# davidfischinger/haf_grasping

Hardware: AMD Instinct MI355X
Metric: grid-cell x rotation SVM evals/sec (higher is better)
Workload: dtype f16

## Files before the change

haf_grasping_amd/capi.py:

```python
import ctypes as C
import os

import numpy as np

HERE = os.path.dirname(os.path.abspath(__file__))
LIB_PATH = os.environ.get("HAF_LIB", os.path.join(HERE, "libhafgrasp.so"))
TESTLIB_PATH = os.environ.get("HAF_TESTLIB", os.path.join(HERE, "libhafgrasp_testing.so"))

HAF_OK, HAF_E_ARG, HAF_E_IO, HAF_E_DEVICE, HAF_E_CAPACITY, HAF_E_BUDGET, HAF_E_INTERNAL = 0, -1, -2, -3, -4, -5, -6
FLAG_KEEP_DEBUG, FLAG_PROFILE, FLAG_FP32_MFMA, FLAG_SPLIT_F16, FLAG_PROBABILITY, FLAG_FULL_RANK = 1, 2, 4, 8, 16, 32
DBG_HEIGHTS, DBG_INTEGRAL, DBG_MASK, DBG_LABELS, DBG_DECISION, DBG_TRANSFORM, DBG_SCREEN_MARGIN, DBG_PROBABILITY, DBG_GRASPSGRID, DBG_ROI = range(10)
SHARD_ROLLS, SHARD_CLOUDS = 0, 1
FRAME_DEPTH_U16, FRAME_DEPTH_F32, FRAME_XYZ_F32 = 0, 1, 2
MAP_NO_CELL = -32768
MAX_LABELS = 4096
STAGES = ["upload", "bin", "integral", "mask", "features", "svm", "refine", "recheck", "vote", "download"]


class Config(C.Structure):
    _fields_ = [("feature_file", C.c_char_p), ("range_file", C.c_char_p), ("model_file", C.c_char_p),
                ("nr_features_without_shaf", C.c_int32), ("grid_h", C.c_int32), ("grid_w", C.c_int32),
                ("n_rolls", C.c_int32), ("roll_step_deg", C.c_int32), ("z_shift", C.c_float),
                ("graspval_top", C.c_int32), ("device", C.c_int32), ("max_clouds", C.c_int32),
                ("max_points", C.c_int64), ("flags", C.c_uint32), ("graspval_th", C.c_int32),
# ... 229 lines not shown
        L.haf_test_roll_geo.argtypes = [C.POINTER(Config), C.POINTER(GraspInput), C.c_int, C.c_void_p, C.c_void_p,
                                        C.c_void_p]
        L.haf_test_finalize.argtypes = [C.POINTER(Config), C.POINTER(GraspInput), C.c_void_p, C.POINTER(GraspOutput)]
        L.haf_test_roll_pose.argtypes = [C.POINTER(Config), C.POINTER(GraspInput), C.c_void_p, C.c_int,
                                         C.POINTER(GraspOutput), C.POINTER(C.c_int32)]
        L.haf_test_mfma_kappa.argtypes = [E, C.c_void_p, C.c_void_p]
        L.haf_test_f16_mfma.argtypes = [C.c_void_p, C.c_void_p, C.c_void_p, C.c_void_p, C.c_int, C.c_int]
        L.haf_test_screen_state.argtypes = [E, C.POINTER(C.c_int), C.POINTER(C.c_int), C.POINTER(C.c_double)]
        L.haf_test_set_screen_inactive.argtypes = [E]
        L.haf_test_check_canaries.argtypes = [C.c_char_p, C.c_int]
        L.haf_test_canary_buffers.argtypes = []
        L.haf_test_poke_flag0_list.argtypes = [E, C.c_int, C.c_int, C.c_int]
        L.haf_test_overflow_stats.argtypes = [E, C.c_void_p]
        L.haf_test_fetch_list.argtypes = [E, C.c_int, C.c_void_p, C.c_int, C.POINTER(C.c_int)]
        L.haf_test_snapshot_screen.argtypes = [E, C.c_int]
        L.haf_test_fetch_snapshot.argtypes = [E, C.c_int, C.c_longlong, C.c_void_p, C.c_longlong, C.POINTER(C.c_longlong)]
        L.haf_test_tier_plan.argtypes = [C.c_void_p, C.c_int, C.c_void_p, C.c_int, C.c_int]
        L.haf_test_revote.argtypes = [E, C.c_void_p, C.c_void_p, C.c_void_p, C.c_void_p, C.c_void_p]
        L.haf_test_last_batch.argtypes = [E, C.POINTER(C.c_int), C.POINTER(C.c_int)]
        L.haf_test_top_merge.argtypes = [C.POINTER(Config), C.POINTER(GraspInput), C.c_int] + [C.c_void_p] * 5 + \
            [C.c_int, C.c_int, C.c_double, C.c_void_p, C.POINTER(C.c_int32), C.POINTER(C.c_int32)]
    return L


def lib():
    global _lib
    if _lib is None:
        _lib = _bind(LIB_PATH, testing=False)
    return _lib

# ... 440 lines not shown
        a, b, c = C.c_int32(), C.c_int32(), C.c_int32()
        self._check(self._L.haf_model_info(self._h, C.byref(a), C.byref(b), C.byref(c)))
        return dict(n_sv=a.value, dim=b.value, n_features=c.value)

    def last_counts(self):
        a, r, b, c = C.c_int64(), C.c_int64(), C.c_int64(), C.c_int64()
        self._check(self._L.haf_last_tiers(self._h, C.byref(a), C.byref(r), C.byref(b), C.byref(c)))
        return dict(n_evals=a.value, n_refined=r.value, n_rechecked=b.value, n_strict=c.value)

    def fetch_list(self, which, cap=1 << 22):
        buf = np.empty(cap, dtype=np.int32)
        n = C.c_int()
        self._check(self._L.haf_test_fetch_list(self._h, which, buf.ctypes.data_as(C.c_void_p), cap, C.byref(n)))
        return buf[:min(n.value, cap)].copy()

    def snapshot_screen(self, on=True):
        self._check(self._L.haf_test_snapshot_screen(self._h, 1 if on else 0))

    def fetch_snapshot(self, which, offset=0, nbytes=None):
        avail = C.c_longlong()
        self._check(self._L.haf_test_fetch_snapshot(self._h, which, 0, None, 0, C.byref(avail)))
        if nbytes is None:
            nbytes = avail.value - offset
        buf = np.empty(max(0, nbytes), dtype=np.uint8)
        if nbytes > 0:
            self._check(self._L.haf_test_fetch_snapshot(self._h, which, offset, buf.ctypes.data_as(C.c_void_p), nbytes, C.byref(avail)))
        return buf

    def revote(self, labels=None, gridf=None, heights=None, roi_words=None):
        H, W = self.cfg.grid_h, self.cfg.grid_w
# ... 373 lines not shown
```

haf_grasping_amd/csrc/engine_request.cpp:

```cpp
#include "engine_state.h"

namespace haf_host {

static double host_kernel_value(const SvmModel &m, const double *xg, int n, int kx)
{
    double acc = 0.0;
    if (m.kernel_type == HAF_KERNEL_RBF) {
        for (int k = 0; k < kx; k++) {
            const double sv = k < m.dim ? m.sv[(size_t)n * m.dim + k] : 0.0;
            const double dd = xg[(size_t)k * 16] - sv;
            acc += dd * dd;
        }
        return std::exp(-m.gamma * acc);
    }
    for (int k = 0; k < kx; k++) {
        const double sv = k < m.dim ? m.sv[(size_t)n * m.dim + k] : 0.0;
        acc += xg[(size_t)k * 16] * sv;
    }
    if (m.kernel_type == HAF_KERNEL_POLY) {
        double tmp = m.gamma * acc + m.coef0, ret = 1.0;
        for (int t = m.degree; t > 0; t /= 2) { if (t % 2 == 1) ret *= tmp; tmp = tmp * tmp; }
        return ret;
    }
    if (m.kernel_type == HAF_KERNEL_SIGMOID) return std::tanh(m.gamma * acc + m.coef0);
// ... 133 lines not shown
    p.i8 = f.i8_active && !f.small_exact && !cr_poly_t1;
    if (p.i8) { p.i8_in = L_FLAG; p.i8_out = L_FLAGI; }
    p.fp64 = f.small_exact ? FP64_SMALL : FP64_MFMA;
    p.fp64_in = p.i8 ? L_FLAGI : L_FLAG;
    p.fp64_out = L_FLAG2;
    p.pass0_out = L_FLAG;
    if (p.path != PATH_SCREEN) return p;

    p.cr = v == SCREEN_CR_EXP || v == SCREEN_CR_POLY;
    p.reuse = f.reuse_operands;
    const bool lr_plain = v == SCREEN_PLAIN && f.lr_plain_available;
    p.lr = (p.cr || lr_plain) && f.large && f.lr_available && f.lr_enabled && !f.fused_pre && f.hw > 8192 && !f.reuse_operands;
    p.sp = p.lr && lr_plain ? SP_LRP : p.cr ? SP_CR : SP_PLAIN;
    if (f.use_t0b && f.cr_available && !f.small_exact && (!p.cr || (p.lr && v == SCREEN_CR_EXP)))
        p.t0b = p.sp == SP_LRP && f.lr_fused && !f.t0b_no_gather ? T0B_GATHER : T0B_FEATURES;
    const bool straight = f.small_exact || f.t1_skip;
    if (p.t0b != T0B_NONE) {
        p.pass0_out = L_FLAG0;
        p.t0b_in = L_FLAG0;
        p.t0b_out = straight ? L_FLAG : L_FLAG0B;
    } else {
        p.pass0_out = straight ? L_FLAG : L_FLAG0;
    }
    p.t1 = !straight;
    if (!p.t1) return p;
    p.t1_in = p.t0b != T0B_NONE ? L_FLAG0B : L_FLAG0;
    p.t1_cnt = list_counter(p.t1_in);
    p.t1_out = L_FLAG;
    p.t1cr = cr_poly_t1;
    p.gate = f.calibrated && f.short_gate && f.n_sv >= kShortGateMinSv && f.evals_cap <= 65536;
// ... 21 lines not shown
    int n_frames = 0;
    FrameDev *h_frames = nullptr;
    const FrameDev *d_frames = nullptr;
    RoiViewDev *h_roi_views = nullptr;
    const RoiViewDev *d_roi_views = nullptr;
    std::vector<LastCall::CloudSrc> src;
    CloudDev *h_clouds = nullptr;
    const CloudDev *d_clouds = nullptr;
    const RollGeo *d_geo = nullptr;
    hipStream_t s = nullptr;
    Dims d{};
    float r_row = 0.0f, r_col = 0.0f;
    long evals_cap = 0, evals_sel = 0;
    bool direct = false, short_request = false, small_exact = false, large = false, fused_pre = false;
    bool i8_used = false, t0b_used = false;
    bool lr_used = false;
    int host_resolved = 0;
};

static int check_request(haf_engine *e, int32_t n_clouds, const haf_cloud *clouds, const haf_grasp_input *in, int32_t roll_first,
                         int32_t roll_count, const haf_roll_record *records, Request &q)
{
    if (!clouds || !in || !records || n_clouds < 1) return fail(e, HAF_E_ARG, "haf_score_rolls: null or empty argument");
    const haf_config &c = e->cfg;
    if (n_clouds > c.max_clouds) return fail(e, HAF_E_CAPACITY, "more clouds than max_clouds");
    if (roll_first < 0 || roll_count < 1 || roll_first + roll_count > c.n_rolls) return fail(e, HAF_E_ARG, "roll range outside [0, n_rolls)");
    if (roll_count > e->max_rolls) return fail(e, HAF_E_CAPACITY, "more rolls in one call than max_rolls_per_call");
    HIPCHK(e, hipSetDevice(c.device));
    q.B = n_clouds;
    q.R = roll_count;
// ... 200 lines not shown
        launch_mask_count_roi(e->d_ii.p, q.d_geo, e->d_roi_cells.p, e->d_mask.p, e->d_rowcount.p, d, s);
    } else {
        launch_mask_count(e->d_ii.p, q.d_geo, e->d_mask.p, e->d_rowcount.p, d, s);
    }
    launch_scan(e->d_rowcount.p, e->d_rowoff.p, e->d_brcount.p, e->d_counters.p, d, s);
    launch_compact(e->d_mask.p, e->d_rowcount.p, e->d_rowoff.p, e->d_evalcell.p, d, s);
    if (q.direct) launch_prob_list(e->d_counters.p, CNT_FLAGGED, e->d_flag_list.p, e->list_cap, s);
    return HAF_OK;
}

static TierFacts tier_facts(const haf_engine *e, const Request &q, int mode, bool reuse_operands)
{
    return TierFacts{e->screen_variant, e->cr_available, e->lr_available, e->lr_enabled, e->lr_plain_available, e->lr_fused,
                     e->use_t0b, e->t1_skip, e->t1_cr_available, e->i8_active, e->calibrated, e->short_gate, e->generic_kernel,
                     e->model.n_sv, test_env("HAF_T0B_NO_GATHER") != nullptr, mode, reuse_operands, q.direct, q.small_exact, q.large,
                     q.fused_pre, (long)q.d.H * q.d.W, q.evals_cap};
}

static void launch_screening(haf_engine *e, const Request &q, const TierPlan &p)
{
    const hipStream_t s = q.s;
    const Dims &d = q.d;
    const long evals_cap = q.evals_cap;
    ScreenParams sp_now = p.sp == SP_LRP ? e->screen_lrp : p.sp == SP_CR ? e->screen_cr : e->screen;
    if (p.sp != SP_LRP) sp_now.cr_poly = e->screen_variant == SCREEN_CR_POLY;
    if (p.lr) { sp_now.lr = 1; sp_now.lr_negflags = e->d_inexact.p; sp_now.lr_iiabs = e->d_iiabs.p; }
    if (!p.reuse)
        launch_features(e->d_ii.p, e->d_evalcell.p, e->d_counters.p, e->d_fd.p, e->d_X.p, e->d_gband.p, d, e->range.lower,
                        e->range.upper, e->svm.neg_gamma2, evals_cap, XMODE_SCREEN, sp_now, nullptr, 0, 0, q.large, q.evals_sel, nullptr, e->d_ax.p, s);
    if (e->snap_on && !p.reuse) {
        const long cap = std::min<long>(evals_cap, e->max_evals_pad);
        e->snap_cap = cap;
        (void)hipMemcpyAsync(e->snap_X.p, e->d_X.p, (size_t)((cap + kTile - 1) / kTile) * (size_t)kS0MatBytes, hipMemcpyDeviceToDevice, s);
        (void)hipMemcpyAsync(e->snap_gband.p, e->d_gband.p, (size_t)cap * kBandFloats * sizeof(float), hipMemcpyDeviceToDevice, s);
        (void)hipMemcpyAsync(e->snap_ax.p, e->d_ax.p, (size_t)cap * sizeof(float), hipMemcpyDeviceToDevice, s);
    }
    char *y_img = reinterpret_cast<char *>(e->d_X.p) + (size_t)(e->max_evals_pad / kTile) * (size_t)kS0MatBytes;
    mark(e, HAF_ST_SVM);
    if (p.lr && !e->lr_fused) launch_project(e->d_X.p, e->d_lr_btiles.p, y_img, e->d_gband.p, e->d_counters.p, evals_cap, s);
    if (p.lr)
        launch_svm_screen_lr(e->lr_fused ? reinterpret_cast<char *>(e->d_X.p) : y_img, e->d_gband.p, e->d_ax.p, e->d_svt_lr.p, e->d_evalcell.p, e->d_counters.p, e->svm, e->d_dec.p, e->d_labels.p,
                             e->d_flag0_words.p, e->d_flag0_wgcount.p, list_buf(e, p.pass0_out), e->flag0_cap, e->d_counters.p, d,
                             evals_cap, e->d_margin.p, e->screen_variant, e->crp, e->lr_band, s, handover_counter(p.pass0_out),
                             e->lr_fused ? e->d_lr_btiles_in.p : nullptr);
    else
        launch_svm_screen(e->d_X.p, e->d_gband.p, e->d_ax.p, p.cr ? e->d_svt0_cr.p : e->d_svt0.p, e->d_evalcell.p, e->d_counters.p, e->svm, e->d_dec.p, e->d_labels.p,
                          e->d_flag0_words.p, e->d_flag0_wgcount.p, list_buf(e, p.pass0_out), e->flag0_cap, e->d_counters.p, d, evals_cap, e->d_margin.p,
                          e->screen_variant, e->crp, s, handover_counter(p.pass0_out), nullptr, CNT_EVALS, CNT_FLAGGED0, e->d_screen_part.p, e->screen_parts);
    mark(e, HAF_ST_REFINE);
    const long list_cap = std::min<long>(e->flag0_cap, evals_cap);
    if (p.t0b == T0B_GATHER) {
        launch_svm_screen_lr(reinterpret_cast<char *>(e->d_X.p), e->d_gband.p, e->d_ax.p, e->d_svt_lr.p, e->d_evalcell.p, e->d_counters.p, e->svm, e->d_dec.p,
                             e->d_labels.p, e->d_flag0_words.p, e->d_flag0_wgcount.p, list_buf(e, p.t0b_out), e->flag0_cap,
                             e->d_counters.p, d, list_cap, e->d_margin.p, SCREEN_CR_EXP, e->crp, e->lr_band, s, handover_counter(p.t0b_out),
                             e->d_lr_btiles_in.p, list_buf(e, p.t0b_in), list_counter(p.t0b_in), CNT_FLAGGED0B);
    } else if (p.t0b == T0B_FEATURES) {
        ScreenParams sp_b = e->screen_cr;
        sp_b.cr_poly = 0;
        launch_features(e->d_ii.p, e->d_evalcell.p, e->d_counters.p, e->d_fd.p, e->d_X1.p, e->d_gband.p, d, e->range.lower,
                        e->range.upper, e->svm.neg_gamma2, list_cap, XMODE_SCREEN, sp_b, list_buf(e, p.t0b_in), list_counter(p.t0b_in), e->flag0_cap,
                        false, list_cap, nullptr, e->d_ax.p, s);
        launch_svm_screen(e->d_X1.p, e->d_gband.p, e->d_ax.p, e->d_svt0_cr.p, e->d_evalcell.p, e->d_counters.p, e->svm, e->d_dec.p, e->d_labels.p,
                          e->d_flag0_words.p, e->d_flag0_wgcount.p, list_buf(e, p.t0b_out), e->flag0_cap, e->d_counters.p, d,
                          list_cap, e->d_margin.p, SCREEN_CR_EXP, e->crp, s, handover_counter(p.t0b_out), list_buf(e, p.t0b_in), list_counter(p.t0b_in),
                          CNT_FLAGGED0B, e->d_screen_part.p, e->screen_parts);
    }
    if (p.gate)
        launch_short_list_gate(e->d_counters.p, list_counter(p.gate_in), list_buf(e, p.gate_in), e->flag0_cap, list_buf(e, p.gate_out),
                               CNT_FLAGGEDI, p.gate_out == L_FLAGI, std::min(kShortListGate, e->flag_cap), s);
    if (!p.t1) return;
// ... 117 lines not shown
    }
    return HAF_OK;
}

static int decide(haf_engine *e, Request &q, int mode, bool reuse_operands)
{
    mark(e, HAF_ST_FEATURES);
    const TierPlan p = plan_tiers(tier_facts(e, q, mode, reuse_operands));
    if (p.path == PATH_SCREEN) {
        q.lr_used = p.lr;
        launch_screening(e, q, p);
    } else {
        launch_first_pass(e, q, p);
    }
    q.t0b_used = p.t0b != T0B_NONE;
    q.i8_used = p.i8;
    mark(e, HAF_ST_RECHECK);
    if (p.fp64 != FP64_NONE) {
        if (p.i8) i8_window(e, q, p, 0);
        fp64_window(e, q, p, 0);
    }
    const int rc = vote_and_wait(e, q);
    if (rc != HAF_OK) return rc;
    return finish_exact_tiers(e, q, p);
}

static int decide_probability(haf_engine *e, Request &q)
{
    const hipStream_t s = q.s;
    const Dims &d = q.d;
// ... 84 lines not shown
}

static int record_outcome(haf_engine *e, const Request &q, int mode, int inexact_grids, int roll_first, const haf_grasp_input *in,
                          haf_roll_record *records)
{
    if (e->cfg.flags & HAF_FLAG_PROFILE)
        for (int i = 0; i < HAF_ST_COUNT; i++) (void)hipEventElapsedTime(&e->stage_ms[i], e->ev[i], e->ev[i + 1]);
    const int *h = e->h_counters;
    LastCall &l = e->last;
    l.B = q.B; l.R = q.R; l.roll_first = roll_first;
    l.evals = h[CNT_EVALS];
    l.flagged = e->prob_mode ? 0 : h[CNT_FLAGGED];
    l.flagged2 = h[CNT_FLAGGED2];
    l.lr = q.lr_used;
    l.flagged0 = q.t0b_used ? std::min(h[CNT_FLAGGED0B], h[CNT_FLAGGED0]) : h[CNT_FLAGGED0];
    l.flaggedi = q.i8_used ? h[CNT_FLAGGEDI] : h[CNT_FLAGGED];
    l.bypass = h[CNT_BYPASS];
    l.inexact = inexact_grids;
    l.screened = (mode == MODE_SCREEN) && !e->prob_mode && !q.direct && h[CNT_FLAGGED0] <= e->flag0_cap;
    l.host_resolved = q.host_resolved;
    l.i8 = q.i8_used;
    l.inputs.assign(in, in + q.B);
    l.clouds = q.src;
    l.roi = q.from.roi != nullptr;
    for (int b = 0; q.from.views && b < q.B; b++) l.clouds[(size_t)b].n = (size_t)q.h_clouds[b].n;
    if (hipMemsetAsync(e->d_counters.p, 0, CNT_COUNT * sizeof(int), q.s) == hipSuccess) e->counters_clean = true;
    if (l.flagged > e->list_cap || l.flagged2 > e->list_cap || l.flaggedi > e->list_cap) return fail(e, HAF_E_INTERNAL, "recheck list counters exceed the number of evaluations");
    if (const int rc = check_guards(e)) return rc;
    for (int i = 0; i < q.B * q.R; i++) {
        records[i].vote = e->h_rec[i].vote;
// ... 116 lines not shown
```

haf_grasping_amd/csrc/engine_state.h:

```cpp
#pragma once
#include "../../include/hafgrasp.h"
#include "kernels.h"
#include "parsers.h"
#include "frame_stage.h"
#include "decq.h"
#include "engine_internal.h"

#include <algorithm>
#include <chrono>
#include <cmath>
#include <cstdio>
#include <cstdlib>
#include <cstring>
#include <mutex>
#include <new>
#include <string>
#include <vector>

using namespace haf;

namespace haf_host {

#ifdef HAF_TESTING
inline const char *test_env(const char *name) { return getenv(name); }
// ... 89 lines not shown
        char *h = nullptr;
        hipError_t rc = d.alloc(bytes);
        pinned_failed = rc == hipSuccess && (rc = hipHostMalloc((void **)&h, bytes, hipHostMallocDefault)) != hipSuccess;
        if (rc != hipSuccess) { d.release(); return rc; }
        release();
        dev = d; host = h;
        return hipSuccess;
    }
    void release() { dev.release(); if (host) (void)hipHostFree(host); host = nullptr; }
};

struct LastCall {
    int B = 0, R = 0, roll_first = 0;
    int evals = 0;
    int flagged0 = 0;
    int flagged = 0;
    int flaggedi = 0;
    int bypass = 0;
    int flagged2 = 0;
    int host_resolved = 0;
    int inexact = 0;
    bool screened = false;
    bool lr = false;
    bool i8 = false;
    std::vector<haf_grasp_input> inputs;
    struct CloudSrc { size_t float_off = 0; size_t n = 0; bool staged = false; };
    std::vector<CloudSrc> clouds;
    bool roi = false;
};

// ... 207 lines not shown
inline int list_counter(int l)
{
    static const int cnt[] = {CNT_FLAGGED0, CNT_FLAGGED0B, CNT_FLAGGED, CNT_FLAGGEDI, CNT_FLAGGED2};
    return l == L_NONE ? -1 : cnt[l];
}
struct TierFacts {
    int screen_variant = SCREEN_PLAIN;
    bool cr_available = false, lr_available = false, lr_enabled = false, lr_plain_available = false, lr_fused = false;
    bool use_t0b = false, t1_skip = false, t1_cr_available = false, i8_active = false, calibrated = false, short_gate = false;
    bool generic_kernel = false;
    int n_sv = 0;
    bool t0b_no_gather = false;
    int mode = MODE_SCREEN;
    bool reuse_operands = false, direct = false, small_exact = false, large = false, fused_pre = false;
    long hw = 0, evals_cap = 0;
};
enum { PATH_GENERIC, PATH_DIRECT, PATH_SCREEN, PATH_SPLIT, PATH_F32 };
enum { SP_PLAIN, SP_CR, SP_LRP };
enum { T0B_NONE, T0B_GATHER, T0B_FEATURES };
enum { FP64_NONE, FP64_SMALL, FP64_MFMA };
struct TierPlan {
    int path = PATH_SCREEN;
    int sp = SP_PLAIN;
    bool cr = false, lr = false;
    bool reuse = false;
    int pass0_out = L_NONE;
    int t0b = T0B_NONE, t0b_in = L_NONE, t0b_out = L_NONE;
    bool gate = false;
    int gate_in = L_NONE, gate_out = L_NONE;
    bool t1 = false, t1cr = false;
    int t1_in = L_NONE, t1_cnt = -1, t1_out = L_NONE;
    bool i8 = false;
    int i8_in = L_NONE, i8_out = L_NONE;
    int fp64 = FP64_NONE, fp64_in = L_NONE, fp64_out = L_NONE;
    int strict_in = L_FLAG2;
};
TierPlan plan_tiers(const TierFacts &f);

inline int fail(haf_engine *e, int code, const std::string &msg)
{
    e->error = msg;
    return code;
// ... 63 lines not shown
```

haf_grasping_amd/csrc/engine_testing.cpp:

```cpp
#include "engine_state.h"

#ifndef HAF_TESTING
#error "engine_testing.cpp belongs to the testing build (-DHAF_TESTING)"
#endif

namespace haf_host {
namespace {
struct CanaryRec { char *user; size_t bytes; const char *file; int line; };
std::mutex g_canary_mu;
std::vector<CanaryRec> g_canary;
}
void canary_register(void *user, size_t bytes, const char *file, int line)
{
    std::lock_guard<std::mutex> lk(g_canary_mu);
    g_canary.push_back(CanaryRec{static_cast<char *>(user), bytes, file, line});
}
void canary_unregister(void *user)
{
    std::lock_guard<std::mutex> lk(g_canary_mu);
    for (size_t i = 0; i < g_canary.size(); i++)
        if (g_canary[i].user == user) { g_canary[i] = g_canary.back(); g_canary.pop_back(); return; }
}
int canary_check(std::string *report)
{
// ... 93 lines not shown
    if (!e || !avail || offset < 0 || bytes < 0 || which < 0 || which > 2) return HAF_E_ARG;
    const char *src = which == 0 ? e->snap_X.p : which == 1 ? reinterpret_cast<const char *>(e->snap_gband.p) : reinterpret_cast<const char *>(e->snap_ax.p);
    const long long have = which == 0 ? (long long)((e->snap_cap + kTile - 1) / kTile) * kS0MatBytes
                                      : (long long)e->snap_cap * (which == 1 ? kBandFloats : 1) * (long long)sizeof(float);
    *avail = src ? have : 0;
    if (!bytes) return HAF_OK;
    if (!src || !out || offset + bytes > have) return HAF_E_ARG;
    if (hipDeviceSynchronize() != hipSuccess) return HAF_E_DEVICE;
    return hipMemcpy(out, src + offset, (size_t)bytes, hipMemcpyDeviceToHost) == hipSuccess ? HAF_OK : HAF_E_DEVICE;
}
int haf_test_poke_flag0_list(haf_engine *e, int at, int count, int v)
{
    if (!e || !e->d_flag0_list.p) return HAF_E_ARG;
    std::vector<int> h((size_t)count, v);
    return hipMemcpy(e->d_flag0_list.p + e->d_flag0_list.n + at, h.data(), h.size() * sizeof(int), hipMemcpyHostToDevice) == hipSuccess ? HAF_OK : HAF_E_DEVICE;
}

int haf_test_last_batch(haf_engine *e, int *B, int *R)
{
    if (!e || !B || !R) return HAF_E_ARG;
    *B = e->last.B; *R = e->last.R;
    return HAF_OK;
}

static int revote_impl(haf_engine *e, const int8_t *labels, const float *gridf, const float *heights, const unsigned long long *roi_words,
                       haf_roll_record *records_out)
{
    if (!records_out || (labels != nullptr) == (gridf != nullptr)) return fail(e, HAF_E_ARG, "haf_test_revote: exactly one of labels and gridf, and records_out");
    if ((gridf != nullptr) != e->prob_mode) return fail(e, HAF_E_ARG, "haf_test_revote: labels go with a plain engine, gridf with HAF_FLAG_PROBABILITY");
    if (roi_words && !labels) return fail(e, HAF_E_ARG, "haf_test_revote: roi_words go with labels");
// ... 355 lines not shown
```

haf_grasping_amd/csrc/kernels.h:

```cpp
#pragma once

#include <hip/hip_runtime.h>
#include <stddef.h>
#include <stdint.h>
#include "frame_points.h"
#include "frames.h"
#include "grasp_cells.h"

namespace haf {

constexpr int kKP = 324;
constexpr int kKSteps = kKP / 2;
constexpr int kDP = 328;
constexpr int kTile = 32;
constexpr int kTileFloats = kDP * kTile;
constexpr int kSvmBlockEvals = 256;
constexpr int kSvmThreads = 512;
constexpr int kHListParts = 4;

constexpr int kHK = 336;
constexpr int kHFull = 10;
constexpr int kHSteps = kHK / 16;
constexpr int kHMatBytes = kHSteps * 1024;
constexpr int kHTailOff = kHFull * 2048;
// ... 13 lines not shown
constexpr int kS0WaveEvals = 64;
constexpr int kS0Waves = 4;
constexpr int kS0BlockEvals = kS0Waves * kS0WaveEvals;
constexpr int kS0K = 320;
constexpr int kS0Groups = kS0K / 8;
constexpr int kS0MatBytes = kHFull * 2048;
constexpr int kS0WavePieces = 5;
constexpr int kS0SvTileBytes = 21504;
constexpr int kS0Pieces = kS0SvTileBytes / 1024;
constexpr int kS0Buffers = 3;
constexpr float kF16MinNormal = 6.103515625e-05f;
constexpr int kLrK = 192;
constexpr int kLrSteps = kLrK / 32;
constexpr int kLrMatBytes = kLrSteps * 2048;
constexpr int kLrSvTileBytes = kLrMatBytes + 1024;
constexpr int kLrWavePieces = 3;
constexpr int kLrProjTileBytes = kHFull * 2048;

__host__ __device__ inline double split3_f16(double a, _Float16 out[3])
{
    auto rn = [](double v) {
        _Float16 h = (_Float16)(float)v;
        float f = (float)h;
        if ((f < 0 ? -f : f) < kF16MinNormal) h = (_Float16)0.0f;
        return h;
    };
    out[0] = rn(a);
    const double r1 = a - (double)(float)out[0];
    out[1] = rn(r1 * 4096.0);
    const double r2 = r1 - (double)(float)out[1] / 4096.0;
// ... 239 lines not shown
       XMODE_F64 = 3,
       XMODE_I8 = 4 };
void launch_features(const float *ii, const int *evalcell, const int *counters, const FeatDesc *fd, float *X, float *ax,
                     Dims d, double lower, double upper, float neg_gamma2, long max_evals, int xmode, ScreenParams sp,
                     const int *idx_list, int list_counter, int list_cap, bool large, long sel_evals, AttrRecord *dbg,
                     float *ax2, hipStream_t s,
                     int list_off = 0);
double probe_mfma_rounding(hipStream_t s, double *worst16);
int probe_f16_subnormal_mfma(hipStream_t s);
void launch_project(const void *X0, const void *btiles, void *Y, float *raw, const int *counters, long max_evals, hipStream_t s);
void launch_svm_screen_lr(const void *Y, float *raw, const float *nax, const void *svt_lr, const int *evalcell, const int *counters,
                          SvmParams p, float *dec, int8_t *labels, unsigned long long *flag0_words, int *wgcount, int *flag0_list,
                          int flag0_cap, int *counters_rw, Dims d, long max_evals, float *margin, int variant, CrParams cr, LrBand lb,
                          hipStream_t s, int also_counter = -1,
                          const void *ptiles = nullptr,
                          const int *idx_list = nullptr, int count_slot = CNT_EVALS, int out_slot = CNT_FLAGGED0);
void launch_svm_screen(const void *X0, const float *gband, const float *nax, const void *svt0, const int *evalcell, const int *counters,
                       SvmParams p, float *dec, int8_t *labels, unsigned long long *flag0_words, int *wgcount, int *flag0_list,
                       int flag0_cap, int *counters_rw, Dims d, long max_evals, float *margin, int variant, CrParams cr, hipStream_t s,
                       int also_counter = -1,
                       const int *idx_list = nullptr, int count_slot = CNT_EVALS,
                       int out_slot = CNT_FLAGGED0,
                       void *part_buf = nullptr, int parts = 0);
size_t screen_part_bytes();
void launch_svm(const float *X, const float *ax, const float *svt, const int *evalcell, const int *counters,
                SvmParams p, float *dec, int8_t *labels, int *flag_list, int flag_cap, int *counters_rw, Dims d,
                long max_evals, hipStream_t s,
                unsigned char *t1flags = nullptr);
void launch_short_list_gate(int *counters, int src_slot, const int *src_list, int src_cap, int *dst_list, int dst_slot, bool dst_direct,
                            int max_entries, hipStream_t s);
size_t t1_flag_bytes(long max_entries);
// ... 113 lines not shown
```

haf_grasping_amd/csrc/screen.hip:

```cpp
#include "kernels.h"
#include "screen_band.h"
#include <algorithm>
#include <cmath>
#include <vector>

namespace haf {

typedef float f32x4 __attribute__((ext_vector_type(4)));
typedef _Float16 half8 __attribute__((ext_vector_type(8)));
typedef _Float16 half4 __attribute__((ext_vector_type(4)));

__device__ __forceinline__ void dma_piece(const char *gbase, unsigned lds_dst, unsigned lane16)
{
    asm volatile("s_mov_b32 m0, %0\n\ts_nop 0\n\tglobal_load_lds_dwordx4 %1, %2" ::"s"(lds_dst), "v"(lane16), "s"(gbase) : "memory", "m0");
}

struct TileDma {
    const char *g[kS0WavePieces];
    unsigned l[kS0WavePieces];
};
__device__ __forceinline__ TileDma tile_dma(const char *gtile, unsigned lds_slot, const int (&poff)[kS0WavePieces])
{
    TileDma d;
#pragma unroll
// ... 744 lines not shown
{
    const long blocks = (max_evals + kS0BlockEvals - 1) / kS0BlockEvals;
    if (blocks <= 0) return;
    hipLaunchKernelGGL(k_project, dim3((unsigned)blocks), dim3(kS0Waves * 64), 0, s, (const char *)X0, (const char *)btiles, (char *)Y, raw, counters);
}

#ifndef HAF_LR_WGS
#define HAF_LR_WGS 2
#endif
#ifndef HAF_LR_EXPLAG
#define HAF_LR_EXPLAG 4
#endif
#ifndef HAF_LR_ABL
#define HAF_LR_ABL 0
#endif
constexpr int kLrExpLag = HAF_LR_EXPLAG;
constexpr bool kLrTwoLevel = HAF_LR_WGS < 3;
template <int FIRST, int COUNT, int VAR>
__device__ __forceinline__ void screen_block_lr(const char *cur, int n, int lane, const half8 (&a)[kLrSteps][4], f32x4 (&acc)[4],
                                                const f32x4 (&old)[4], float cf_old, float (&sum)[4][4],
                                                const TileDma &dma, unsigned lane16, half8 &b, half8 &b1)
{
    constexpr bool CRP = VAR == SCREEN_CR_POLY, PLN = VAR == SCREEN_PLAIN;
    static_assert(VAR == SCREEN_CR_EXP || VAR == SCREEN_CR_POLY || VAR == SCREEN_PLAIN, "the low-rank form serves the plain and the centred-remainder variants");
    const char *bl = cur + n * 1024 + lane * 16;
    __builtin_amdgcn_sched_barrier(0);
    const f32x4 z4 = {0.0f, 0.0f, 0.0f, 0.0f};
    const float ba2 = CRP ? cf_old * kPsiA2 : 0.0f, ba3 = CRP ? cf_old * kPsiA3 : 0.0f, ba4 = CRP ? cf_old * kPsiA4 : 0.0f;
    if (n == 0) b = *reinterpret_cast<const half8 *>(bl);
    if (HAF_LR_ABL & 2) asm volatile("" :: "v"(old[0]), "v"(old[1]), "v"(old[2]), "v"(old[3]));
// ... 38 lines not shown
                float ph = fmaf(z, ba4, ba3);
                HAF_SB();
                ph = fmaf(ph, z, ba2);
                HAF_SB();
                sum[e >> 2][e & 3] = fmaf(pt, ph, sum[e >> 2][e & 3]);
                HAF_SB();
            }
        }
        b = b1;
    }
#undef HAF_SB
    __builtin_amdgcn_sched_barrier(0);
}

template <int VAR, bool FUSED, bool GATHER>
__global__ __launch_bounds__(kS0Waves * 64, HAF_LR_WGS) void k_svm_screen_lr(const char *__restrict__ Y, const float *__restrict__ raw,
                                                                  const float *__restrict__ nax, const char *__restrict__ svt,
                                                                  const int *__restrict__ evalcell, const int *__restrict__ counters,
                                                                  SvmParams p, float *__restrict__ dec, int8_t *__restrict__ labels,
                                                                  unsigned long long *__restrict__ flag0_words, Dims d,
                                                                  float *__restrict__ margin, CrParams crp, LrBand lb,
                                                                  const char *__restrict__ ptiles,
                                                                  const int *__restrict__ idx_list, int count_slot, int in_cap)
{
    static_assert(!GATHER || FUSED, "the gather form reads the 10-step images");
    constexpr bool CRP = VAR == SCREEN_CR_POLY;
    constexpr int kV0 = FUSED ? kHFull : 0;
    __shared__ __attribute__((aligned(16))) char lds[kS0Buffers * kLrSvTileBytes + 3 * kS0Waves * kS0WaveEvals * 4];
    const int n_evals = GATHER ? min(counters[count_slot], in_cap) : counters[CNT_EVALS];
    const long base = (long)blockIdx.x * kS0BlockEvals;
    if (base >= n_evals) return;
    const int tid = threadIdx.x, wave = tid >> 6, lane = tid & 63;
    const long tile32 = (base >> 5) + 2 * wave;
    const unsigned lds0 = (unsigned)(uintptr_t)lds;
    const int np = d.sv_tile_neg, nt = d.n_sv_tiles;
    float *pos = reinterpret_cast<float *>(lds + kS0Buffers * kLrSvTileBytes) + wave * kS0WaveEvals;
    float *fin = pos + kS0Waves * kS0WaveEvals;
    float *sdyrow = fin + kS0Waves * kS0WaveEvals;
    const unsigned lane16 = (unsigned)lane * 16u;
    const int wave_u = __builtin_amdgcn_readfirstlane(wave);
    int poff[kS0WavePieces];
// ... 4 lines not shown
        asm volatile("s_nop 4");
#pragma unroll
        for (int q = 0; q < kLrWavePieces; q++) dma_piece(g + poff[q], l + (unsigned)poff[q], lane16);
    };
    auto vtile = [&](int v) -> const char * { return (FUSED && v < kV0) ? ptiles + (size_t)v * kLrMatBytes : svt + (size_t)(v - kV0) * kLrSvTileBytes; };
    {
        stage3(vtile(0), lds0);
        if (!FUSED && wave_u == 0) dma_piece(svt + kLrMatBytes, lds0 + kLrMatBytes, lane16);
    }
    if (FUSED || nt > 1) {
        stage3(vtile(1), lds0 + kLrSvTileBytes);
        if (!FUSED && wave_u == 0) dma_piece(vtile(1) + kLrMatBytes, lds0 + kLrSvTileBytes + kLrMatBytes, lane16);
    }
    half8 a[kLrSteps][4];
    if (!FUSED) {
        const char *xt = Y + (size_t)tile32 * kLrMatBytes;
#pragma unroll
        for (int s = 0; s < kLrSteps; s++)
#pragma unroll
            for (int m = 0; m < 4; m++)
                a[s][m] = __builtin_nontemporal_load(reinterpret_cast<const half8 *>(xt + (m >> 1) * kLrMatBytes + (s * 2 + (m & 1)) * 1024 + lane * 16));
#pragma unroll
        for (int s = 0; s < kLrSteps; s++)
#pragma unroll
            for (int m = 0; m < 4; m++) asm volatile("" : "+v"(a[s][m]));
        asm volatile("s_waitcnt vmcnt(0)" ::: "memory");
        __syncthreads();
    } else {
        const char *xt = Y + (size_t)tile32 * kS0MatBytes;
        const char *xg[4];
        if (GATHER) {
#pragma unroll
            for (int m = 0; m < 4; m++) {
                const long sl = base + wave * kS0WaveEvals + 16 * m + (lane & 15);
                const int eg = sl < n_evals ? idx_list[sl] : 0;
                xg[m] = Y + (size_t)(eg >> 5) * kS0MatBytes + ((eg >> 4) & 1) * 1024 + ((lane >> 4) * 16 + (eg & 15)) * 16;
            }
        }
        auto xload = [&](int sx, half8 (&x)[4]) {
#pragma unroll
            for (int m = 0; m < 4; m++)
                x[m] = GATHER ? *reinterpret_cast<const half8 *>(xg[m] + sx * 2048)
                              : __builtin_nontemporal_load(reinterpret_cast<const half8 *>(xt + (m >> 1) * kS0MatBytes + (sx * 2 + (m & 1)) * 1024 + lane * 16));
        };
        f32x4 accp[2 * kLrSteps][4];
#pragma unroll
        for (int rb = 0; rb < 2 * kLrSteps; rb++)
#pragma unroll
            for (int m = 0; m < 4; m++) accp[rb][m] = f32x4{0.0f, 0.0f, 0.0f, 0.0f};
        half8 xc[4], xn[4];
        xload(0, xc);
#pragma unroll
        for (int m = 0; m < 4; m++) xn[m] = xc[m];
#pragma unroll
        for (int m = 0; m < 4; m++) asm volatile("" : "+v"(xc[m]));
        asm volatile("s_waitcnt vmcnt(0)" ::: "memory");
        __syncthreads();
#pragma unroll 1
        for (int v = 0; v < kV0; v++) {
            const char *cur = lds + (v % kS0Buffers) * kLrSvTileBytes;
#pragma unroll
            for (int rb = 0; rb < 2 * kLrSteps; rb++) {
                const half8 bf = *reinterpret_cast<const half8 *>(cur + rb * 1024 + lane * 16);
                if (!(HAF_LR_ABL & 16)) {
#pragma unroll
                for (int m = 0; m < 4; m++) accp[rb][m] = __builtin_amdgcn_mfma_f32_16x16x32_f16(bf, xc[m], accp[rb][m], 0, 0, 0);
                } else if (rb < 4) {
                    accp[rb][0] = __builtin_amdgcn_mfma_f32_16x16x32_f16(bf, xc[rb], accp[rb][0], 0, 0, 0);
                }
                if (rb == 0) {
                    __builtin_amdgcn_sched_barrier(0);
                    if (v + 1 < kV0) xload(v + 1, xn);
                    const int vn = v + 2;
                    if (vn < kV0 + nt) {
                        const unsigned ls = lds0 + (vn % kS0Buffers) * kLrSvTileBytes;
                        stage3(vtile(vn), ls);
                        if (vn >= kV0 && wave_u == 0) dma_piece(vtile(vn) + kLrMatBytes, ls + kLrMatBytes, lane16);
                    }
                    __builtin_amdgcn_sched_barrier(0);
// ... 112 lines not shown
        const long es = GATHER ? (long)idx_list[e] : e;
        float sc = __builtin_amdgcn_exp2f(nax[es]);
        float4 g, g2 = float4{0.0f, 0.0f, 0.0f, 0.0f};
        float rw[6];
#pragma unroll
        for (int k = 0; k < 6; k++) rw[k] = raw[kBandFloats * es + k];
        if (GATHER) rw[3] = raw[kBandFloats * es + 6];
        if (FUSED) rw[5] = sdyrow[lane];
        if (VAR == SCREEN_PLAIN) lr_finish_band_plain(rw, lb, g, g2);
        else lr_finish_band(rw, lb, g.x, g.y, g.z, g.w);
        asm volatile("s_nop 7\n\ts_nop 7" : "+v"(sc));
        flagged = screen_tail_vals<VAR, false>((double)pos[lane], (double)fin[lane], 0.0f, e, g, g2, sc, p, crp, GATHER ? idx_list : nullptr, evalcell, dec, labels, margin);
    }
    const unsigned long long bal = __ballot(flagged);
    if (lane == 0) flag0_words[(base >> 6) + wave] = bal;
}

void launch_svm_screen(const void *X0, const float *gband, const float *nax, const void *svt0, const int *evalcell, const int *counters,
                       SvmParams p, float *dec, int8_t *labels, unsigned long long *flag0_words, int *wgcount, int *flag0_list,
                       int flag0_cap, int *counters_rw, Dims d, long max_evals, float *margin, int variant, CrParams cr, hipStream_t s,
                       int also_counter, const int *idx_list, int count_slot, int out_slot, void *part_buf, int parts)
{
    long blocks = (max_evals + kS0BlockEvals - 1) / kS0BlockEvals;
    if (blocks <= 0) return;
    const int in_cap = idx_list ? (int)std::min<long>(flag0_cap, max_evals) : 0x7fffffff;
    const bool split = part_buf && parts != 1 && blocks <= kS0PartBlocks && (parts > 1 || d.n_sv_tiles >= 4 * kS0MinPartTiles);
#define HAF_SCREEN_LAUNCH(V)                                                                                                      \
    if (split) {                                                                                                                  \
        hipLaunchKernelGGL((k_svm_screen<V, true>), dim3((unsigned)blocks, kS0MaxParts), dim3(kS0Waves * 64), 0, s, (const char *)X0, gband, nax, \
                           (const char *)svt0, evalcell, counters, p, dec, labels, flag0_words, d, margin, cr, idx_list, count_slot,      \
// ... 6 lines not shown
                           (float4 *)nullptr, 0, in_cap);                                                                         \
    }
    switch (variant) {
        case SCREEN_SUMSQ: HAF_SCREEN_LAUNCH(SCREEN_SUMSQ); break;
        case SCREEN_CR_EXP: HAF_SCREEN_LAUNCH(SCREEN_CR_EXP); break;
        case SCREEN_CR_POLY: HAF_SCREEN_LAUNCH(SCREEN_CR_POLY); break;
        default: HAF_SCREEN_LAUNCH(SCREEN_PLAIN); break;
    }
#undef HAF_SCREEN_LAUNCH
    launch_screen_compaction(flag0_words, wgcount, blocks, flag0_list, flag0_cap, counters_rw, also_counter, idx_list, count_slot, out_slot, in_cap, s);
}

void launch_svm_screen_lr(const void *Y, float *raw, const float *nax, const void *svt_lr, const int *evalcell, const int *counters,
                          SvmParams p, float *dec, int8_t *labels, unsigned long long *flag0_words, int *wgcount, int *flag0_list,
                          int flag0_cap, int *counters_rw, Dims d, long max_evals, float *margin, int variant, CrParams cr, LrBand lb,
                          hipStream_t s, int also_counter, const void *ptiles, const int *idx_list, int count_slot, int out_slot)
{
    const long blocks = (max_evals + kS0BlockEvals - 1) / kS0BlockEvals;
    if (blocks <= 0) return;
    lb.poly = variant == SCREEN_CR_POLY;
    const int in_cap = idx_list ? (int)std::min<long>(flag0_cap, max_evals) : 0x7fffffff;
#define HAF_LR_LAUNCH(V, F, G)                                                                                                        \
    hipLaunchKernelGGL((k_svm_screen_lr<V, F, G>), dim3((unsigned)blocks), dim3(kS0Waves * 64), 0, s, (const char *)Y, raw, nax,        \
                       (const char *)svt_lr, evalcell, counters, p, dec, labels, flag0_words, d, margin, cr, lb, (const char *)ptiles,  \
                       idx_list, count_slot, in_cap)
    if (idx_list) { HAF_LR_LAUNCH(SCREEN_CR_EXP, true, true); }
    else if (variant == SCREEN_CR_POLY) { if (ptiles) HAF_LR_LAUNCH(SCREEN_CR_POLY, true, false); else HAF_LR_LAUNCH(SCREEN_CR_POLY, false, false); }
    else if (variant == SCREEN_PLAIN) { if (ptiles) HAF_LR_LAUNCH(SCREEN_PLAIN, true, false); else HAF_LR_LAUNCH(SCREEN_PLAIN, false, false); }
    else { if (ptiles) HAF_LR_LAUNCH(SCREEN_CR_EXP, true, false); else HAF_LR_LAUNCH(SCREEN_CR_EXP, false, false); }
#undef HAF_LR_LAUNCH
    const int cs = idx_list ? count_slot : CNT_EVALS;
    launch_screen_compaction(flag0_words, wgcount, blocks, flag0_list, flag0_cap, counters_rw, also_counter, idx_list, cs,
                             idx_list ? out_slot : CNT_FLAGGED0, in_cap, s);
}

size_t screen_part_bytes() { return (size_t)kS0MaxParts * kS0PartBlocks * kS0BlockEvals * sizeof(float4); }

}
```

Measured before the change: 540.0 million.

## Store first-pass projected LR features for flagged evals and reuse them in second tier

In the fused plain low-rank screen, each wave now writes its projected f16 feature vectors (and a band value) into a per-eval record buffer, but only for evaluations the first pass flags. The second-tier gather pass then reads these compact records instead of re-gathering from the full 10-step images and re-running the projection MFMAs. The aim is to cut the redundant projection work and bandwidth in the refine screen. In exchange the first pass does extra scattered stores, and it relies on the record buffer aliasing the y_img region. Test hooks and a HAF_T0B_REPROJECT escape are also added.

```diff
diff --git a/haf_grasping_amd/capi.py b/haf_grasping_amd/capi.py
--- a/haf_grasping_amd/capi.py
+++ b/haf_grasping_amd/capi.py
@@ -267,6 +267,8 @@
         L.haf_test_overflow_stats.argtypes = [E, C.c_void_p]
         L.haf_test_fetch_list.argtypes = [E, C.c_int, C.c_void_p, C.c_int, C.POINTER(C.c_int)]
         L.haf_test_snapshot_screen.argtypes = [E, C.c_int]
+        L.haf_test_t0b_state.argtypes = [E, C.c_void_p]
+        L.haf_test_fill_lr_records.argtypes = [E, C.c_int]
         L.haf_test_fetch_snapshot.argtypes = [E, C.c_int, C.c_longlong, C.c_void_p, C.c_longlong, C.POINTER(C.c_longlong)]
         L.haf_test_tier_plan.argtypes = [C.c_void_p, C.c_int, C.c_void_p, C.c_int, C.c_int]
         L.haf_test_revote.argtypes = [E, C.c_void_p, C.c_void_p, C.c_void_p, C.c_void_p, C.c_void_p]
@@ -737,6 +739,14 @@
         self._check(self._L.haf_test_fetch_list(self._h, which, buf.ctypes.data_as(C.c_void_p), cap, C.byref(n)))
         return buf[:min(n.value, cap)].copy()
 
+    def t0b_state(self):
+        out = (C.c_int * 3)()
+        self._check(self._L.haf_test_t0b_state(self._h, out))
+        return dict(first_pass_flagged=int(out[0]), form=("none", "gather", "features")[out[1]], stored=bool(out[2]))
+
+    def fill_lr_records(self, byte=0xFF):
+        self._check(self._L.haf_test_fill_lr_records(self._h, byte))
+
     def snapshot_screen(self, on=True):
         self._check(self._L.haf_test_snapshot_screen(self._h, 1 if on else 0))
 
diff --git a/haf_grasping_amd/csrc/engine_request.cpp b/haf_grasping_amd/csrc/engine_request.cpp
--- a/haf_grasping_amd/csrc/engine_request.cpp
+++ b/haf_grasping_amd/csrc/engine_request.cpp
@@ -171,6 +171,7 @@
     p.sp = p.lr && lr_plain ? SP_LRP : p.cr ? SP_CR : SP_PLAIN;
     if (f.use_t0b && f.cr_available && !f.small_exact && (!p.cr || (p.lr && v == SCREEN_CR_EXP)))
         p.t0b = p.sp == SP_LRP && f.lr_fused && !f.t0b_no_gather ? T0B_GATHER : T0B_FEATURES;
+    p.t0b_stored = p.t0b == T0B_GATHER && !f.t0b_reproject;
     const bool straight = f.small_exact || f.t1_skip;
     if (p.t0b != T0B_NONE) {
         p.pass0_out = L_FLAG0;
@@ -222,6 +223,8 @@
     long evals_cap = 0, evals_sel = 0;
     bool direct = false, short_request = false, small_exact = false, large = false, fused_pre = false;
     bool i8_used = false, t0b_used = false;
+    int t0b_form = T0B_NONE;
+    bool t0b_stored = false;
     bool lr_used = false;
     int host_resolved = 0;
 };
@@ -452,7 +455,7 @@
     return TierFacts{e->screen_variant, e->cr_available, e->lr_available, e->lr_enabled, e->lr_plain_available, e->lr_fused,
                      e->use_t0b, e->t1_skip, e->t1_cr_available, e->i8_active, e->calibrated, e->short_gate, e->generic_kernel,
                      e->model.n_sv, test_env("HAF_T0B_NO_GATHER") != nullptr, mode, reuse_operands, q.direct, q.small_exact, q.large,
-                     q.fused_pre, (long)q.d.H * q.d.W, q.evals_cap};
+                     q.fused_pre, (long)q.d.H * q.d.W, q.evals_cap, test_env("HAF_T0B_REPROJECT") != nullptr};
 }
 
 static void launch_screening(haf_engine *e, const Request &q, const TierPlan &p)
@@ -474,13 +477,14 @@
         (void)hipMemcpyAsync(e->snap_ax.p, e->d_ax.p, (size_t)cap * sizeof(float), hipMemcpyDeviceToDevice, s);
     }
     char *y_img = reinterpret_cast<char *>(e->d_X.p) + (size_t)(e->max_evals_pad / kTile) * (size_t)kS0MatBytes;
+    static_assert(kLrRecBytes * kTile == kLrMatBytes, "an evaluation's record is its share of a 6-step image");
     mark(e, HAF_ST_SVM);
     if (p.lr && !e->lr_fused) launch_project(e->d_X.p, e->d_lr_btiles.p, y_img, e->d_gband.p, e->d_counters.p, evals_cap, s);
     if (p.lr)
         launch_svm_screen_lr(e->lr_fused ? reinterpret_cast<char *>(e->d_X.p) : y_img, e->d_gband.p, e->d_ax.p, e->d_svt_lr.p, e->d_evalcell.p, e->d_counters.p, e->svm, e->d_dec.p, e->d_labels.p,
                              e->d_flag0_words.p, e->d_flag0_wgcount.p, list_buf(e, p.pass0_out), e->flag0_cap, e->d_counters.p, d,
                              evals_cap, e->d_margin.p, e->screen_variant, e->crp, e->lr_band, s, handover_counter(p.pass0_out),
-                             e->lr_fused ? e->d_lr_btiles_in.p : nullptr);
+                             e->lr_fused ? e->d_lr_btiles_in.p : nullptr, nullptr, CNT_EVALS, CNT_FLAGGED0, p.t0b_stored ? y_img : nullptr);
     else
         launch_svm_screen(e->d_X.p, e->d_gband.p, e->d_ax.p, p.cr ? e->d_svt0_cr.p : e->d_svt0.p, e->d_evalcell.p, e->d_counters.p, e->svm, e->d_dec.p, e->d_labels.p,
                           e->d_flag0_words.p, e->d_flag0_wgcount.p, list_buf(e, p.pass0_out), e->flag0_cap, e->d_counters.p, d, evals_cap, e->d_margin.p,
@@ -491,7 +495,7 @@
         launch_svm_screen_lr(reinterpret_cast<char *>(e->d_X.p), e->d_gband.p, e->d_ax.p, e->d_svt_lr.p, e->d_evalcell.p, e->d_counters.p, e->svm, e->d_dec.p,
                              e->d_labels.p, e->d_flag0_words.p, e->d_flag0_wgcount.p, list_buf(e, p.t0b_out), e->flag0_cap,
                              e->d_counters.p, d, list_cap, e->d_margin.p, SCREEN_CR_EXP, e->crp, e->lr_band, s, handover_counter(p.t0b_out),
-                             e->d_lr_btiles_in.p, list_buf(e, p.t0b_in), list_counter(p.t0b_in), CNT_FLAGGED0B);
+                             e->d_lr_btiles_in.p, list_buf(e, p.t0b_in), list_counter(p.t0b_in), CNT_FLAGGED0B, p.t0b_stored ? y_img : nullptr);
     } else if (p.t0b == T0B_FEATURES) {
         ScreenParams sp_b = e->screen_cr;
         sp_b.cr_poly = 0;
@@ -639,6 +643,8 @@
         launch_first_pass(e, q, p);
     }
     q.t0b_used = p.t0b != T0B_NONE;
+    q.t0b_form = p.t0b;
+    q.t0b_stored = p.t0b_stored;
     q.i8_used = p.i8;
     mark(e, HAF_ST_RECHECK);
     if (p.fp64 != FP64_NONE) {
@@ -753,6 +759,9 @@
     l.flagged2 = h[CNT_FLAGGED2];
     l.lr = q.lr_used;
     l.flagged0 = q.t0b_used ? std::min(h[CNT_FLAGGED0B], h[CNT_FLAGGED0]) : h[CNT_FLAGGED0];
+    l.pass0_flagged = h[CNT_FLAGGED0];
+    l.t0b_form = q.t0b_form;
+    l.t0b_stored = q.t0b_stored;
     l.flaggedi = q.i8_used ? h[CNT_FLAGGEDI] : h[CNT_FLAGGED];
     l.bypass = h[CNT_BYPASS];
     l.inexact = inexact_grids;
diff --git a/haf_grasping_amd/csrc/engine_state.h b/haf_grasping_amd/csrc/engine_state.h
--- a/haf_grasping_amd/csrc/engine_state.h
+++ b/haf_grasping_amd/csrc/engine_state.h
@@ -127,6 +127,9 @@
     int B = 0, R = 0, roll_first = 0;
     int evals = 0;
     int flagged0 = 0;
+    int pass0_flagged = 0;
+    int t0b_form = 0;
+    bool t0b_stored = false;
     int flagged = 0;
     int flaggedi = 0;
     int bypass = 0;
@@ -364,6 +367,7 @@
     int mode = MODE_SCREEN;
     bool reuse_operands = false, direct = false, small_exact = false, large = false, fused_pre = false;
     long hw = 0, evals_cap = 0;
+    bool t0b_reproject = false;
 };
 enum { PATH_GENERIC, PATH_DIRECT, PATH_SCREEN, PATH_SPLIT, PATH_F32 };
 enum { SP_PLAIN, SP_CR, SP_LRP };
@@ -376,6 +380,7 @@
     bool reuse = false;
     int pass0_out = L_NONE;
     int t0b = T0B_NONE, t0b_in = L_NONE, t0b_out = L_NONE;
+    bool t0b_stored = false;
     bool gate = false;
     int gate_in = L_NONE, gate_out = L_NONE;
     bool t1 = false, t1cr = false;
diff --git a/haf_grasping_amd/csrc/engine_testing.cpp b/haf_grasping_amd/csrc/engine_testing.cpp
--- a/haf_grasping_amd/csrc/engine_testing.cpp
+++ b/haf_grasping_amd/csrc/engine_testing.cpp
@@ -131,6 +131,21 @@
     if (!e || !e->d_flag0_list.p) return HAF_E_ARG;
     std::vector<int> h((size_t)count, v);
     return hipMemcpy(e->d_flag0_list.p + e->d_flag0_list.n + at, h.data(), h.size() * sizeof(int), hipMemcpyHostToDevice) == hipSuccess ? HAF_OK : HAF_E_DEVICE;
+}
+
+int haf_test_t0b_state(haf_engine *e, int *out3)
+{
+    if (!e || !out3) return HAF_E_ARG;
+    out3[0] = e->last.pass0_flagged; out3[1] = e->last.t0b_form; out3[2] = e->last.t0b_stored ? 1 : 0;
+    return HAF_OK;
+}
+int haf_test_fill_lr_records(haf_engine *e, int byte)
+{
+    if (!e || !e->d_X.p) return HAF_E_ARG;
+    char *y_img = reinterpret_cast<char *>(e->d_X.p) + (size_t)(e->max_evals_pad / kTile) * (size_t)kS0MatBytes;
+    if (hipDeviceSynchronize() != hipSuccess) return HAF_E_DEVICE;
+    if (hipMemset(y_img, byte, (size_t)e->max_evals_pad * kLrRecBytes) != hipSuccess) return HAF_E_DEVICE;
+    return hipDeviceSynchronize() == hipSuccess ? HAF_OK : HAF_E_DEVICE;
 }
 
 int haf_test_last_batch(haf_engine *e, int *B, int *R)
diff --git a/haf_grasping_amd/csrc/kernels.h b/haf_grasping_amd/csrc/kernels.h
--- a/haf_grasping_amd/csrc/kernels.h
+++ b/haf_grasping_amd/csrc/kernels.h
@@ -51,6 +51,7 @@
 constexpr int kLrSteps = kLrK / 32;
 constexpr int kLrMatBytes = kLrSteps * 2048;
 constexpr int kLrSvTileBytes = kLrMatBytes + 1024;
+constexpr int kLrRecBytes = kLrSteps * 64;
 constexpr int kLrWavePieces = 3;
 constexpr int kLrProjTileBytes = kHFull * 2048;
 
@@ -320,7 +321,8 @@
                           int flag0_cap, int *counters_rw, Dims d, long max_evals, float *margin, int variant, CrParams cr, LrBand lb,
                           hipStream_t s, int also_counter = -1,
                           const void *ptiles = nullptr,
-                          const int *idx_list = nullptr, int count_slot = CNT_EVALS, int out_slot = CNT_FLAGGED0);
+                          const int *idx_list = nullptr, int count_slot = CNT_EVALS, int out_slot = CNT_FLAGGED0,
+                          void *records = nullptr);
 void launch_svm_screen(const void *X0, const float *gband, const float *nax, const void *svt0, const int *evalcell, const int *counters,
                        SvmParams p, float *dec, int8_t *labels, unsigned long long *flag0_words, int *wgcount, int *flag0_list,
                        int flag0_cap, int *counters_rw, Dims d, long max_evals, float *margin, int variant, CrParams cr, hipStream_t s,
diff --git a/haf_grasping_amd/csrc/screen.hip b/haf_grasping_amd/csrc/screen.hip
--- a/haf_grasping_amd/csrc/screen.hip
+++ b/haf_grasping_amd/csrc/screen.hip
@@ -782,6 +782,9 @@
 #ifndef HAF_LR_ABL
 #define HAF_LR_ABL 0
 #endif
+#ifndef HAF_T0B_ABL
+#define HAF_T0B_ABL 0
+#endif
 constexpr int kLrExpLag = HAF_LR_EXPLAG;
 constexpr bool kLrTwoLevel = HAF_LR_WGS < 3;
 template <int FIRST, int COUNT, int VAR>
@@ -850,17 +853,18 @@
 }
 
 template <int VAR, bool FUSED, bool GATHER>
-__global__ __launch_bounds__(kS0Waves * 64, HAF_LR_WGS) void k_svm_screen_lr(const char *__restrict__ Y, const float *__restrict__ raw,
+__global__ __launch_bounds__(kS0Waves * 64, HAF_LR_WGS) void k_svm_screen_lr(const char *__restrict__ Y, float *__restrict__ raw,
                                                                   const float *__restrict__ nax, const char *__restrict__ svt,
                                                                   const int *__restrict__ evalcell, const int *__restrict__ counters,
                                                                   SvmParams p, float *__restrict__ dec, int8_t *__restrict__ labels,
                                                                   unsigned long long *__restrict__ flag0_words, Dims d,
                                                                   float *__restrict__ margin, CrParams crp, LrBand lb,
                                                                   const char *__restrict__ ptiles,
-                                                                  const int *__restrict__ idx_list, int count_slot, int in_cap)
-{
-    static_assert(!GATHER || FUSED, "the gather form reads the 10-step images");
+                                                                  const int *__restrict__ idx_list, int count_slot, int in_cap,
+                                                                  char *__restrict__ rec)
+{
     constexpr bool CRP = VAR == SCREEN_CR_POLY;
+    constexpr bool STORE = VAR == SCREEN_PLAIN && FUSED && !GATHER;
     constexpr int kV0 = FUSED ? kHFull : 0;
     __shared__ __attribute__((aligned(16))) char lds[kS0Buffers * kLrSvTileBytes + 3 * kS0Waves * kS0WaveEvals * 4];
     const int n_evals = GATHER ? min(counters[count_slot], in_cap) : counters[CNT_EVALS];
@@ -895,12 +899,26 @@
     }
     half8 a[kLrSteps][4];
     if (!FUSED) {
+        if (GATHER) {
+#pragma unroll
+            for (int m = 0; m < 4; m++) {
+                const long sl = base + wave * kS0WaveEvals + 16 * m + (lane & 15);
+#pragma unroll
+                for (int s = 0; s < kLrSteps; s++) a[s][m] = half8{0, 0, 0, 0, 0, 0, 0, 0};
+                if (sl < n_evals) {
+                    const char *r = Y + (size_t)idx_list[sl] * kLrRecBytes + (lane >> 4) * 16;
+#pragma unroll
+                    for (int s = 0; s < kLrSteps; s++) a[s][m] = *reinterpret_cast<const half8 *>(r + s * 64);
+                }
+            }
+        } else {
         const char *xt = Y + (size_t)tile32 * kLrMatBytes;
 #pragma unroll
         for (int s = 0; s < kLrSteps; s++)
 #pragma unroll
             for (int m = 0; m < 4; m++)
                 a[s][m] = __builtin_nontemporal_load(reinterpret_cast<const half8 *>(xt + (m >> 1) * kLrMatBytes + (s * 2 + (m & 1)) * 1024 + lane * 16));
+        }
 #pragma unroll
         for (int s = 0; s < kLrSteps; s++)
 #pragma unroll
@@ -914,7 +932,7 @@
 #pragma unroll
             for (int m = 0; m < 4; m++) {
                 const long sl = base + wave * kS0WaveEvals + 16 * m + (lane & 15);
-                const int eg = sl < n_evals ? idx_list[sl] : 0;
+                const int eg = (sl < n_evals && !(HAF_T0B_ABL & 2)) ? idx_list[sl] : 0;
                 xg[m] = Y + (size_t)(eg >> 5) * kS0MatBytes + ((eg >> 4) & 1) * 1024 + ((lane >> 4) * 16 + (eg & 15)) * 16;
             }
         }
@@ -943,7 +961,7 @@
 #pragma unroll
             for (int rb = 0; rb < 2 * kLrSteps; rb++) {
                 const half8 bf = *reinterpret_cast<const half8 *>(cur + rb * 1024 + lane * 16);
-                if (!(HAF_LR_ABL & 16)) {
+                if (!(HAF_LR_ABL & 16) && !(GATHER && (HAF_T0B_ABL & 1))) {
 #pragma unroll
                 for (int m = 0; m < 4; m++) accp[rb][m] = __builtin_amdgcn_mfma_f32_16x16x32_f16(bf, xc[m], accp[rb][m], 0, 0, 0);
                 } else if (rb < 4) {
@@ -1086,6 +1104,18 @@
     }
     const unsigned long long bal = __ballot(flagged);
     if (lane == 0) flag0_words[(base >> 6) + wave] = bal;
+    if constexpr (STORE) {
+        if (rec != nullptr && bal != 0ull) {
+            if (flagged) raw[kBandFloats * e + 5] = sdyrow[lane];
+            char *rq = rec + (size_t)(base + wave * kS0WaveEvals + (lane & 15)) * kLrRecBytes + (lane >> 4) * 16;
+#pragma unroll
+            for (int m = 0; m < 4; m++)
+                if ((bal >> (16 * m + (lane & 15))) & 1ull) {
+#pragma unroll
+                    for (int s = 0; s < kLrSteps; s++) *reinterpret_cast<half8 *>(rq + (size_t)(16 * m) * kLrRecBytes + s * 64) = a[s][m];
+                }
+        }
+    }
 }
 
 void launch_svm_screen(const void *X0, const float *gband, const float *nax, const void *svt0, const int *evalcell, const int *counters,
@@ -1122,7 +1152,7 @@
 void launch_svm_screen_lr(const void *Y, float *raw, const float *nax, const void *svt_lr, const int *evalcell, const int *counters,
                           SvmParams p, float *dec, int8_t *labels, unsigned long long *flag0_words, int *wgcount, int *flag0_list,
                           int flag0_cap, int *counters_rw, Dims d, long max_evals, float *margin, int variant, CrParams cr, LrBand lb,
-                          hipStream_t s, int also_counter, const void *ptiles, const int *idx_list, int count_slot, int out_slot)
+                          hipStream_t s, int also_counter, const void *ptiles, const int *idx_list, int count_slot, int out_slot, void *records)
 {
     const long blocks = (max_evals + kS0BlockEvals - 1) / kS0BlockEvals;
     if (blocks <= 0) return;
@@ -1131,8 +1161,10 @@
 #define HAF_LR_LAUNCH(V, F, G)                                                                                                        \
     hipLaunchKernelGGL((k_svm_screen_lr<V, F, G>), dim3((unsigned)blocks), dim3(kS0Waves * 64), 0, s, (const char *)Y, raw, nax,        \
                        (const char *)svt_lr, evalcell, counters, p, dec, labels, flag0_words, d, margin, cr, lb, (const char *)ptiles,  \
-                       idx_list, count_slot, in_cap)
-    if (idx_list) { HAF_LR_LAUNCH(SCREEN_CR_EXP, true, true); }
+                       idx_list, count_slot, in_cap, rec)
+    char *rec = idx_list ? nullptr : (char *)records;
+    if (idx_list && records) { Y = records; HAF_LR_LAUNCH(SCREEN_CR_EXP, false, true); }
+    else if (idx_list) { HAF_LR_LAUNCH(SCREEN_CR_EXP, true, true); }
     else if (variant == SCREEN_CR_POLY) { if (ptiles) HAF_LR_LAUNCH(SCREEN_CR_POLY, true, false); else HAF_LR_LAUNCH(SCREEN_CR_POLY, false, false); }
     else if (variant == SCREEN_PLAIN) { if (ptiles) HAF_LR_LAUNCH(SCREEN_PLAIN, true, false); else HAF_LR_LAUNCH(SCREEN_PLAIN, false, false); }
     else { if (ptiles) HAF_LR_LAUNCH(SCREEN_CR_EXP, true, false); else HAF_LR_LAUNCH(SCREEN_CR_EXP, false, false); }
```

New measurement: 539.8 million. About the same (-0.0%).
